# TUM-AVS/Frenetix-Motion-Planner

Measured on AMD Instinct MI355X. Metric: candidate trajectories/sec (30-step horizon), higher is better.
Workload: dtype f64; 1 GPU; BASELINE config3: single agent, 50388 candidates/GPU x 31 samples (19x51x52 grid per GPU), 20 predicted obstacles (prediction cost + OBB collision), SoA TrajectoryBundle materialised (Mode B); candidates_global=50388, candidates_per_gpu=50388, samples=31, reference_knots=400, obstacles=20, parallelism=single GPU, exchange=none (one rank)

## Files before the change

frenetix-motion-planner_amd/csrc/fx_api.hip:

```cpp
#include "fx_context.h"

thread_local char g_err[512] = "";

extern "C" int32_t fx_wait_word(const volatile unsigned long long *word, unsigned long long expected, int32_t timeout_ms) {
    if (!word) return set_err(FX_ERR_INVALID_ARGUMENT, "fx_wait_word: NULL argument");
    for (int spin = 0; spin < 4096; spin++)
        if (__atomic_load_n(word, __ATOMIC_ACQUIRE) == expected) return FX_OK;
    const auto t0 = std::chrono::steady_clock::now();
    const auto limit = std::chrono::milliseconds(timeout_ms < 0 ? 0 : timeout_ms);
    for (;;) {
        for (int spin = 0; spin < 1024; spin++)
            if (__atomic_load_n(word, __ATOMIC_ACQUIRE) == expected) return FX_OK;
        if (std::chrono::steady_clock::now() - t0 >= limit)
            return set_err(FX_ERR_TIMEOUT, "no answer from the device within %d ms (a peer that never joined the collective, or a "
                           "faulted kernel)", timeout_ms);
    }
}

extern "C" {


int32_t fx_abi_version(void) { return FX_ABI_VERSION; }
const char *fx_last_error(void) { return g_err; }

// ... 285 lines not shown
    const int n = (int)std::min<long long>(have, max_n);
    for (int k = 0; k < n; k++) {
        FxContext::TimeSlot &t = c->ring[(c->n_timed - n + k) % FxContext::kTimeRing];
        int rc = fetch_slot(c, t);
        if (rc) return rc;
        if (obst_ms) obst_ms[k] = t.obst_ms;
    }
    *n_out = n;
    return FX_OK;
}
int32_t fx_step_info_ex(const FxContext *c, int64_t *out16) {
    if (!c || !out16) return set_err(FX_ERR_INVALID_ARGUMENT, "fx_step_info_ex: NULL argument");
    int rc = fx_step_info(c, out16);
    if (rc) return rc;
    out16[10] = c->split_step; out16[11] = c->split_CH; out16[12] = c->obs_blocks_step; out16[13] = (int64_t)c->obs_lds_step;
    out16[14] = c->obs_wg_step; out16[15] = c->tail_step | ((int64_t)c->stage_path << 8);
    if (c->step_kernel_step) {
        out16[11] = c->step_CH; out16[12] = (int64_t)c->step_blocks * (FX_BLOCK / 64); out16[13] = (int64_t)c->step_lds; out16[14] = 0;
        out16[15] |= 1 << 16;
    }
    return FX_OK;
}

int32_t fx_set_step_kernel(FxContext *c, int32_t mode, int32_t steps_per_item) {
    if (!c) return set_err(FX_ERR_INVALID_ARGUMENT, "context is NULL");
    if (mode < 0 || mode > 2) return set_err(FX_ERR_INVALID_ARGUMENT, "mode must be 0 (auto), 1 (off: three launches) or 2 (on where applicable)");
    if (steps_per_item != 0 && steps_per_item != 3 && steps_per_item != 5 && steps_per_item != 8)
        return set_err(FX_ERR_INVALID_ARGUMENT, "steps_per_item must be 0 (auto), 3, 5 or 8");
    c->step_kernel_force = mode; c->step_kernel_CH = steps_per_item;
    return FX_OK;
}
// ... 25 lines not shown
```

frenetix-motion-planner_amd/csrc/fx_api_exchange.hip:

```cpp
#include "fx_context.h"

extern "C" {

namespace {
struct Rccl {
    typedef struct { char internal[128]; } UniqueId;
    int (*GetUniqueId)(UniqueId *) = nullptr;
    int (*CommInitRank)(void **, int, UniqueId, int) = nullptr;
    int (*CommDestroy)(void *) = nullptr;
    int (*AllGather)(const void *, void *, size_t, int, void *, hipStream_t) = nullptr;
    int (*CommCount)(void *, int *) = nullptr;
    const char *(*GetErrorString)(int) = nullptr;
    bool ok = false;
};
Rccl *rccl() {
    static Rccl r;
    static std::once_flag once;
    std::call_once(once, [] {
        void *h = dlopen("librccl.so.1", RTLD_NOW | RTLD_LOCAL);
        if (!h) h = dlopen("librccl.so", RTLD_NOW | RTLD_LOCAL);
        if (h) {
            r.GetUniqueId = reinterpret_cast<decltype(r.GetUniqueId)>(dlsym(h, "ncclGetUniqueId"));
            r.CommInitRank = reinterpret_cast<decltype(r.CommInitRank)>(dlsym(h, "ncclCommInitRank"));
            r.CommDestroy = reinterpret_cast<decltype(r.CommDestroy)>(dlsym(h, "ncclCommDestroy"));
// ... 204 lines not shown
    keep_hip(hipSetDevice(c->device), "hipSetDevice");
    if (total > c->gather_cap) {
        double *bigger = nullptr;
        if (hipStreamSynchronize(c->stream) == hipSuccess && hipMalloc(reinterpret_cast<void **>(&bigger), sizeof(double) * (size_t)FX_PUB_MAX) == hipSuccess) {
            if (c->d_gather) { (void)hipFree(c->d_gather); c->dev_bytes -= (int64_t)(sizeof(double) * c->gather_cap); }
            c->d_gather = bigger; c->gather_cap = FX_PUB_MAX; c->dev_bytes += (int64_t)(sizeof(double) * (size_t)FX_PUB_MAX);
        } else {
            (void)hipGetLastError();
            return set_err(FX_ERR_HIP, "fx_step_exchange_topk: no memory for the %zu-element receive buffer", (size_t)FX_PUB_MAX);
        }
    }
    if (c->n_agents > A) keep(set_err(FX_ERR_CAPACITY, "%d uploaded agents but the communicator exchanges %d rows per rank (fx_comm_set_agents)", c->n_agents, A));
    long long *send_idx = reinterpret_cast<long long *>(c->d_xsend + (size_t)A * k);
    bool evaluated = false;
    if (!rc_local) {
        const int rc = fx_evaluate(c);
        keep(rc);
        if (rc == FX_OK) {
            const hipError_t e = fx_launch_topk(c->d_probs, c->n_agents, max_candidates_of(c), k, c->d_topk_scr_cost, c->d_topk_scr_idx, c->d_xsend, send_idx, c->stream);
            keep_hip(e, "fx_launch_topk");
            evaluated = e == hipSuccess;
        }
    }
    const int n_mine = evaluated ? c->n_agents : 0;
    if (c->comm_k_clean != k || c->comm_rows_clean > n_mine) {
        keep_hip(fill_no_survivor(c, n_mine, k), "hipMemcpyAsync");
        c->comm_k_clean = k;
    }
    c->comm_rows_clean = n_mine;
    RCCL_TRY(rccl()->AllGather(c->d_xsend, exchange_recv(c), n,  8, c->comm, c->stream));
    int rc;
// ... 15 lines not shown
```

frenetix-motion-planner_amd/csrc/fx_api_step.hip:

```cpp
#include "fx_context.h"

extern "C" {

int32_t fx_upload_batch(FxContext *c, int32_t n_agents, const FxProblem *probs) {
    if (!c || !probs) return set_err(FX_ERR_INVALID_ARGUMENT, "fx_upload: NULL argument");
    if (n_agents < 1 || n_agents > c->max_agents) return set_err(FX_ERR_CAPACITY, "n_agents=%d exceeds capacity %d", n_agents, c->max_agents);
    if (c->timed_out) return set_err(FX_ERR_TIMEOUT, "an earlier wait on this context timed out (its stream may never drain): destroy it");
    HIP_TRY(hipSetDevice(c->device));
    if (c->in_flight) {
        { HIP_TRY(hipStreamSynchronize(c->stream)); c->tail_work = c->user_stream; }
        c->in_flight = false;
    }
    c->uploaded = c->evaluated = false;
    Arena ar{c->h_in, c->d_in, c->probs_bytes, c->in_bytes};
    size_t bound_need = 0;
    for (int a = 0; a < n_agents; a++) {
        const FxProblem *p = &probs[a];
        if ((p->mode & FX_MODE_ROAD_BOUNDARY) && p->n_bound > 0 && p->bound_bin && p->M > 0)
            bound_need += align_up(sizeof(double) * 4 * (size_t)p->n_bound, 256) + align_up(sizeof(int32_t) * ((size_t)p->M + 1), 256) +
                          align_up(sizeof(int32_t) * (size_t)std::max(p->bound_bin[p->M], 0), 256);
        if (p->n_lane > 0 && p->lane_poly_off && p->lane_ctr_off)
            bound_need += align_up(sizeof(double) * 4 * (size_t)p->n_lane, 256) + 2 * align_up(sizeof(int32_t) * ((size_t)p->n_lane + 1), 256) +
                          align_up(sizeof(double) * 2 * (size_t)std::max(p->lane_poly_off[p->n_lane], 0), 256) +
                          align_up(sizeof(double) * 2 * (size_t)std::max(p->lane_ctr_off[p->n_lane], 0), 256);
// ... 268 lines not shown
            const size_t rb = sizeof(double) * (size_t)S_rec_doubles(S, std::max(p->K, 0));
            if (!deferred && p->K > 0 && p->K <= 64 && rb <= FX_REC_LDS_MAX && (rec_rule_grid || rec_rule_gen)) d.mode |= FX_MODE_INT_REC_LDS;
        }
        all_deferred = all_deferred && deferred;
        if (deferred) {
            d.mode |= FX_MODE_INT_DEFER_OBST;
            const int n_tiles = (int)((C + 63) / 64), NC = (S - 1 + c->split_CH - 1) / c->split_CH;
            const int NC_alloc = std::max(NC, (S - 1 + 2) / 3);
            d.n_blocks = n_tiles;
            c->obs_blocks_step = std::max(c->obs_blocks_step, n_tiles * NC);
            c->obs_tiles_step = std::max(c->obs_tiles_step, n_tiles);
            c->obs_wg_waves = std::max(c->obs_wg_waves, NC);
            d.obs_part = reinterpret_cast<double *>(obs_part_need);
            d.obs_colm = reinterpret_cast<unsigned long long *>(obs_colm_need);
            d.obs_ticket = reinterpret_cast<unsigned int *>(obs_tick_need);
            obs_part_need += (size_t)NC_alloc * (size_t)ld;
            obs_colm_need += (size_t)NC_alloc * (size_t)n_tiles;
            obs_tick_need += (size_t)n_tiles;
        }
        if (block_off + d.n_blocks > c->max_blocks_total)
            return set_err(FX_ERR_CAPACITY, "agent %d: %lld workgroups exceed the partial-result capacity %lld", a,
                           (long long)(block_off + d.n_blocks), (long long)c->max_blocks_total);
        d.part_cost = c->d_part_cost + block_off;
        d.part_idx = c->d_part_idx + block_off;
        d.counters = c->d_counters + (size_t)a * FX_CNT_COUNT;
        d.pkg_out = c->h_pkg_dev + (size_t)a * c->pkg_stride;
        d.pkg_seq = reinterpret_cast<unsigned long long *>(d.pkg_out + c->pkg_stride - 1);
        d.pkg_plane_rows = c->pkg_plane_rows;
        if (d.mode & FX_MODE_WRITE_BUNDLE) {
            if ((uint64_t)ld * 8u >= (1ull << 32))
                return set_err(FX_ERR_CAPACITY, "agent %d: %lld candidates with a materialised bundle (rows are limited to 4 GiB)", a, (long long)C);
// ... 49 lines not shown
            HIP_TRY(hipMemsetAsync(c->d_obs_ticket, 0, sizeof(unsigned int) * n_tick, c->stream));
        }
        if (!c->d_obs_list) {
            int rc;
            if ((rc = dev_alloc(c, &c->d_obs_list, (size_t)c->total_ld))) return rc;
        }
        for (int a = 0; a < n_agents; a++) {
            DevProblem &d = c->h_probs[a];
            if (!(d.mode & FX_MODE_INT_DEFER_OBST)) continue;
            d.obs_part = c->d_obs_part + reinterpret_cast<size_t>(d.obs_part);
            d.obs_colm = c->d_obs_colm + reinterpret_cast<size_t>(d.obs_colm);
            d.obs_ticket = c->d_obs_ticket + reinterpret_cast<size_t>(d.obs_ticket);
            d.obs_list = c->d_obs_list + (d.cost - c->d_cost);
        }
    }
    c->step_kernel_ok = c->step_kernel_force == 2 && c->split_step && all_deferred && c->use_grid && c->G_step == 2 && c->wsplit_step &&
                        c->block_step == FX_BLOCK && c->wpe_step == 2 && c->any_bundle && !c->any_obst && !c->any_extra && c->wt_step &&
                        c->obs_blocks_step > 0 && c->K_max_step <= 64;
    c->last_live = -1;
    c->n_agents = n_agents;
    c->in_used = ar.off;
    c->dirty_lo = (size_t)-1; c->dirty_hi = 0; c->probs_dirty = false;
    {
        const size_t up = (ar.off + 15) & ~(size_t)15;
        if (up <= c->in_bytes && host_stage_allowed(c, up))
            host_stage(c, 0, up);
        else if (c->stage_mode == 2 || (c->stage_mode != 1 && up <= FX_STAGE_KERNEL_MAX && up <= c->in_bytes)) {
            HIP_TRY(fx_launch_stage(c->h_in_dev, c->d_in, up, c->stream));
            c->stage_path = 2;
        } else {
// ... 44 lines not shown
    if (timed && !attached) HIP_TRY(hipEventRecord(ts->e0, c->stream));
    c->seq++;
    c->fused_step = c->fuse_enabled && c->fusable_step && c->eval_launched;
    c->pkg_step = c->package_enabled && c->any_bundle;
    double *winner = c->dev_winner ? c->dev_winner : (c->pkg_step ? c->d_winner_own : nullptr);
    const bool tail_kernel = FX_TAIL_IN_KERNEL(c->G_step, c->any_extra);
    if (c->fused_step && c->count_step && !tail_kernel) c->fused_step = false;
    c->tail_step = 0;
    if (c->fused_step && tail_kernel) {
        if (c->count_step) c->tail_step |= FX_TAIL_COUNT;
        if (c->pkg_step && c->wt_step) c->tail_step |= FX_TAIL_PACKAGE;
    }
    const bool pkg_in_tail = (c->tail_step & FX_TAIL_PACKAGE) != 0;
    FuseArgs fuse{c->fused_step ? c->h_counters_dev : nullptr, c->seq, winner, (int32_t)((uint32_t)c->K_max_step | (c->tail_step << 16))};
    c->step_kernel_step = false;
    if (c->step_kernel_ok && !c->fused_step && c->eval_launched) {
        int64_t c_max = 0;
        for (int a = 0; a < c->n_agents; a++) c_max = std::max(c_max, c->slots[a].C);
        const int64_t live_est = c->last_live >= 0 ? std::min(c->last_live, c_max) : (2 * c_max + 2) / 3;
        const int tiles_est = (int)std::max<int64_t>(1, (live_est + 63) / 64);
        int best_CH = 0, best_blocks = 0, best_score = 1 << 30;
        size_t best_lds = 0;
        static const int chs[3] = {3, 5, 8};
        for (int q = 0; q < 3; q++) {
            const int CH = chs[q];
            if (c->step_kernel_CH && c->step_kernel_CH != CH) continue;
            const size_t lds = std::max(c->lds_step, (size_t)(FX_BLOCK / 64) * sizeof(double) * 6 * (size_t)CH * (size_t)c->K_max_step);
            int cap = 0;
            {
                static std::mutex mu;
// ... 43 lines not shown
        else
            HIP_TRY(fx_launch_eval(c->d_probs, c->n_agents, c->max_blocks_step,
                                   sizeof(double) * ((size_t)c->M_max_step * FX_REF_FIELDS + FX_TP * (size_t)c->S_max_step +
                                                     (((size_t)c->M_max_step + 1) & ~(size_t)1)) + c->gen_rec_lds,
                                   c->G_step, c->any_bundle, c->any_obst, c->any_extra, c->wpe_step, k0, k1, fuse, c->stream));
    }
    if (timed && !attached) HIP_TRY(hipEventRecord(ts->e_eval, c->stream));
    if (timed) ts->obst_timed = false;
    if (c->split_step && c->obs_blocks_step > 0) {
        const bool t_obs = timed && c->timing == FX_TIMING_KERNEL;
        const char *wg_env = getenv("FX_OBST_WG");
        const int wg_mode = wg_env ? (atoi(wg_env) ? 2 : 1) : ((int64_t)c->obs_tiles_step * c->n_agents <= 1024 ? 2 : 1);
        const size_t lds_wg = align_up((size_t)c->obs_wg_waves * (c->obs_lds_step + 64 * sizeof(double) + sizeof(unsigned long long)), 16);
        const bool wg = wg_mode == 2 && c->obs_wg_waves >= 1 && c->obs_wg_waves <= 16 && lds_wg <= (size_t)160 * 1024 - 1024;
        c->obs_wg_step = wg ? c->obs_wg_waves : 0;
        HIP_TRY(fx_launch_obstacle(c->d_probs, c->n_agents, c->obs_blocks_step, wg ? lds_wg : c->obs_lds_step, c->split_CH,
                                   t_obs ? ts->e_obs0 : nullptr, t_obs ? ts->e_obs1 : nullptr, c->stream, wg ? c->obs_wg_waves : 0,
                                   c->obs_tiles_step));
        if (timed) ts->obst_timed = t_obs;
    }
    if (!c->fused_step) {
        int64_t c_max = 0;
        for (int a = 0; a < c->n_agents; a++) c_max = std::max(c_max, c->slots[a].C);
        HIP_TRY(fx_launch_select(c->d_probs, c->n_agents, c_max, c->h_counters_dev, c->seq, winner, c->pkg_step ? c->h_pkg_dev : nullptr,
                                 c->pkg_stride, c->pkg_plane_rows, c->stream));
    } else if (c->pkg_step && !pkg_in_tail) {
        HIP_TRY(fx_launch_package(c->d_probs, c->n_agents, winner, c->h_pkg_dev, c->pkg_stride, c->pkg_plane_rows, c->seq, c->stream));
    }
    const bool one_launch = c->fused_step && (!c->pkg_step || pkg_in_tail);
    if (timed && !one_launch) HIP_TRY(hipEventRecord(ts->e_end, c->stream));
    if (timed) { ts->fused = one_launch; c->n_timed++; }
    c->timed_step = timed;
    c->evaluated = true;
    c->in_flight = true;
    return FX_OK;
}
// ... 274 lines not shown
```

frenetix-motion-planner_amd/csrc/fx_context.h:

```cpp
#pragma once

#include <hip/hip_runtime.h>

#include <algorithm>
#include <chrono>
#include <cmath>
#include <cstdarg>
#include <cstdio>
#include <cstdlib>
#include <cstring>
#include <atomic>

#include <map>
#include <memory>
#include <mutex>
#include <new>
#include <thread>
#include <tuple>
#include <vector>
#include <dlfcn.h>
#include <fcntl.h>
#include <unistd.h>

#include "fx_device.h"

extern "C" hipError_t fx_launch_eval(const DevProblem *d_probs, int n_agents, int max_blocks, size_t lds_bytes, int G,
                                     bool bundle, bool obst, bool extra, int wpe, hipEvent_t ev_start, hipEvent_t ev_stop,
                                     FuseArgs fuse, hipStream_t stream);
extern "C" hipError_t fx_launch_eval_grid(const DevProblem *d_probs, int n_agents, int max_blocks, int block_size,
                                          size_t lds_bytes, int G, bool bundle, bool obst, int wpe, bool wsplit,
                                          hipEvent_t ev_start, hipEvent_t ev_stop, FuseArgs fuse, hipStream_t stream);
extern "C" hipError_t fx_launch_obstacle(const DevProblem *d_probs, int n_agents, int max_items, size_t lds_bytes, int CH,
                                         hipEvent_t ev_start, hipEvent_t ev_stop, hipStream_t stream, int wg_waves, int max_tiles);
extern "C" hipError_t fx_step_kernel_capacity(int CH, size_t lds_bytes, int *blocks_out);
extern "C" hipError_t fx_launch_step(const DevProblem *d_probs, int n_agents, int blocks, size_t lds_bytes, int CH, hipEvent_t ev_start,
                                     hipEvent_t ev_stop, FuseArgs fuse, StepArgs sa, hipStream_t stream);
extern "C" hipError_t fx_launch_select(const DevProblem *d_probs, int n_agents, int64_t max_candidates, unsigned long long *host_result,
                                       unsigned long long seq, double *dev_winner, double *host_pkg, int pkg_stride, int pkg_plane_rows,
                                       hipStream_t stream);
extern "C" hipError_t fx_launch_math_test(int n, const double *x, double *at, double *sn, double *cs, hipStream_t stream);
extern "C" hipError_t fx_launch_publish(const double *src, int n, double *host_dst, unsigned long long *host_seq,
                                        unsigned long long seq, hipStream_t stream);
extern "C" hipError_t fx_launch_stage(const void *src_mapped, void *dst, size_t bytes, hipStream_t stream);
extern "C" hipError_t fx_launch_package(const DevProblem *d_probs, int n_agents, const double *winner, double *host_pkg, int stride,
                                        int plane_rows, unsigned long long seq, hipStream_t stream);
extern "C" hipError_t fx_launch_topk(const DevProblem *d_probs, int n_agents, int64_t max_candidates, int k, double *scr_cost, long long *scr_idx,
                                     double *out_cost, long long *out_idx, hipStream_t stream);

// ... 124 lines not shown
    size_t in_used = 0;
    size_t dirty_lo = (size_t)-1, dirty_hi = 0;
    bool probs_dirty = false;
    int max_blocks_step = 0, M_max_step = 0, S_max_step = 0, K_max_step = 0;
    int G_step = 1, wpe_step = 2;
    int G_force = 0, wpe_force = 0;
    int variant_force = 0;
    int block_force = 0;
    int wsplit_force = 0;
    int obst_force = 0;
    int obst_CH = 0;
    bool split_step = false;
    int split_CH = 3, obs_blocks_step = 0;
    int obs_wg_waves = 0, obs_tiles_step = 0;
    int obs_wg_step = 0;
    size_t obs_lds_step = 0;
    int step_kernel_force = 0;
    int step_kernel_CH = 0;
    bool step_kernel_ok = false;
    bool step_kernel_step = false;
    int step_blocks = 0, step_CH = 0;
    size_t step_lds = 0;
    int64_t last_live = -1;
    unsigned long long *d_bar = nullptr;
    unsigned long long bar_base = 0;
    int store_force = 0;
    bool wsplit_step = false;
    int block_step = FX_BLOCK;
    bool use_grid = false;
    size_t lds_step = 0;
// ... 262 lines not shown
```

frenetix-motion-planner_amd/csrc/fx_device.h:

```cpp
#pragma once
#include <hip/hip_runtime.h>
#include <stdint.h>

#include "../../include/fxplan.h"

#define FX_BLOCK 256
#define FX_MODE_INT_STORE_WT (1u << 30)
#define FX_MODE_INT_DEFER_OBST (1u << 29)
#define FX_MODE_INT_REC_LDS (1u << 28)
#define FX_HOT_STRIDE 10
#define FX_HOT_PRE 4
#define FX_TP 14
#define FX_REF_FIELDS 8
#define FX_MAX_SAMPLES 128
#define FX_REC_LDS_MAX (48 * 1024)
__host__ __device__ inline int S_rec_doubles(int S, int K) { return S * K * 12; }

struct DevProblem {
    int32_t N, S;
    uint32_t mode;
    int32_t low_vel_mode;
    double dt;
    double x0_lon[3], x0_lat[3];
    double x0_orientation, v_des;
// ... 165 lines not shown
#define FX_MSTAMP(k) do { } while (0)
#endif

#define FX_COEFF_ROWS 13
#define FX_PKG_TAIL (12 + FX_NUM_COSTS + 6)

enum {
    FX_CNT_RETURNED = 0, FX_CNT_FEASIBLE, FX_CNT_HIST0,
    FX_CNT_BEST_IDX = FX_CNT_HIST0 + FX_NUM_REASONS, FX_CNT_BEST_COST, FX_CNT_COLLISIONS, FX_CNT_COUNT
};

#define FX_DCNT_TICKET FX_CNT_BEST_IDX
#define FX_DCNT_LIVE FX_CNT_BEST_COST
#define FX_TAIL_COUNT 1u
#define FX_TAIL_PACKAGE 2u
#define FX_TAIL_IN_KERNEL(G, EXTRA) ((G) >= 4 || (EXTRA))
struct FuseArgs {
    unsigned long long *host_result;
    unsigned long long seq;
    double *dev_winner;
    int32_t k_max;
    __host__ __device__ uint32_t tail() const { return (uint32_t)k_max >> 16; }
    __host__ __device__ int32_t kmax() const { return k_max & 0xffff; }
};

struct StepArgs {
    unsigned long long *bar;
    unsigned long long bar_base;
    unsigned long long *host_result;
    unsigned long long seq;
// ... 22 lines not shown
```

frenetix-motion-planner_amd/csrc/fx_kernels.hip:

```cpp
#include <hip/hip_ext.h>

#include <atomic>

#include "fx_eval_kernel.h"
#include "fx_eval_grid_kernel.h"
#include "fx_obstacle_kernel.h"
#include "fx_step_kernel.h"
#include "fx_risk_kernel.h"

using fxk::wave_count;

#if defined(__HIP_DEVICE_COMPILE__) && !defined(__gfx950__) && !defined(__gfx942__) && !defined(__gfx90a__)
#error "libfxplan's kernels are written for gfx950 (row_bcast DPP controls, wave64): build with --offload-arch=gfx950"
#endif

#define FX_MAX_DEVICES 64
static inline int fx_device_slot() {
    int d = 0;
    if (hipGetDevice(&d) != hipSuccess || d < 0) d = 0;
    return d % FX_MAX_DEVICES;
}

#ifdef FX_CULL_STATS
__device__ unsigned long long fx_cull_stats[16];
// ... 395 lines not shown
    }
    switch (G) {
    case 32: FX_BO(32, 2, false);
    case 16: FX_BO(16, 2, false);
    case 8: FX_W(8, false);
    case 4: FX_W(4, false);
    case 2: FX_W(2, false);
    default: FX_W(1, false);
    }
#undef FX_W
#undef FX_BO
#undef FX_LAUNCH
}

extern "C" hipError_t fx_launch_obstacle(const DevProblem *d_probs, int n_agents, int max_items, size_t lds_bytes, int CH,
                                         hipEvent_t ev_start, hipEvent_t ev_stop, hipStream_t stream, int wg_waves, int max_tiles) {
#define FX_LAUNCH(CHv)                                                                                                                \
    do {                                                                                                                            \
        if (wg_waves > 0) {                                                                                                         \
            static std::atomic<size_t> lds_set_[FX_MAX_DEVICES];                                                                    \
            std::atomic<size_t> &hw_ = lds_set_[fx_device_slot()];                                                                  \
            if (lds_bytes > 48 * 1024 && lds_bytes > hw_.load(std::memory_order_relaxed)) {                                         \
                hipError_t e_ = hipFuncSetAttribute(reinterpret_cast<const void *>(&fxk::fx_obstacle_kernel<CHv, 4, true>),          \
                                                    hipFuncAttributeMaxDynamicSharedMemorySize, (int)lds_bytes);                    \
                if (e_ != hipSuccess) return e_;                                                                                    \
                hw_.store(lds_bytes, std::memory_order_relaxed);                                                                    \
            }                                                                                                                       \
            hipExtLaunchKernelGGL((fxk::fx_obstacle_kernel<CHv, 4, true>), dim3(max_tiles, n_agents), dim3(64 * wg_waves), lds_bytes, stream, \
                                  ev_start, ev_stop, 0, d_probs);                                                                   \
        } else {                                                                                                                    \
            hipExtLaunchKernelGGL((fxk::fx_obstacle_kernel<CHv, 4, false>), dim3(max_items, n_agents), dim3(64), lds_bytes, stream, ev_start, \
                                  ev_stop, 0, d_probs);                                                                             \
        }                                                                                                                           \
        return hipGetLastError();                                                                                                   \
    } while (0)
    if (CH == 2) FX_LAUNCH(2);
    if (CH == 3) FX_LAUNCH(3);
    if (CH == 5) FX_LAUNCH(5);
#undef FX_LAUNCH
    return hipErrorInvalidValue;
}

#define FX_STEP_CASES(X) X(3) X(5) X(8)
extern "C" hipError_t fx_step_kernel_capacity(int CH, size_t lds_bytes, int *blocks_out) {
    int dev = 0, cus = 0, per_cu = 0;
    hipError_t e = hipGetDevice(&dev);
    if (e != hipSuccess) return e;
// ... 69 lines not shown
```

frenetix-motion-planner_amd/csrc/fx_obstacle_kernel.h:

```cpp
#pragma once

#include "fx_eval_kernel.h"

namespace fxk {

struct ObsEntry {
    double l11, l12, l22;
    fx_d2 cc;
};
template <class HotPtr>
__device__ __forceinline__ ObsEntry obs_load(HotPtr hot_i, const fx_d2 *cc_i, int k) {
    const auto q = hot_i + (size_t)k * FX_HOT_STRIDE;
    ObsEntry e;
    e.l11 = q[FX_HOT_L11]; e.l12 = q[FX_HOT_L12]; e.l22 = q[FX_HOT_L22];
    e.cc = cc_i[k];
    return e;
}
__device__ __forceinline__ double obs_msq(const ObsEntry &e, double xr, double yr) {
    const double u = fma(e.l11, xr, fma(e.l12, yr, -e.cc.x));
    const double w = fma(e.l22, yr, -e.cc.y);
    const double m = fma(u, u, w * w);
    return m * m;
}
__device__ __forceinline__ double obs_four(double a, double b, double c, double d) {
    const double ab = a * b, cd = c * d;
    const double num = fma(a + b, cd, (c + d) * ab);
    return num * rcp_pred(ab * cd);
}

#ifndef FX_OBST_WG_WPE
#define FX_OBST_WG_WPE 1
#endif
template <int CH, bool WG, bool COH>
__device__ __forceinline__ void fx_obstacle_body(const DevProblem &P, double *__restrict__ lds_all, const int tile, const int chunk,
                                                 const long long n_live_known = -1) {
    static_assert(!COH || !WG, "the one-launch step runs single-wave items");
    auto LD = [](auto p) { return *p; };
    auto ST = [](auto p, auto v) { if (COH) st_agent(p, v); else *p = v; };
    const uint32_t mode = P.mode;
    if (!(mode & FX_MODE_INT_DEFER_OBST)) return;
    const int S = P.S, K = P.K;
    const int NC = (S - 1 + CH - 1) / CH;
    const int64_t C = P.C, ld = P.ld;
    const int n_wave = WG ? (int)(blockDim.x >> 6) : 1;
    const int64_t c0 = (int64_t)tile * 64;
    if (c0 >= C) return;
    const int lane = threadIdx.x & 63;
    double *__restrict__ lds_dyn = lds_all + (WG ? (size_t)chunk * 6 * CH * (size_t)K : 0);
    double *__restrict__ sh_part = lds_all + (size_t)n_wave * 6 * CH * (size_t)K;
    unsigned long long *__restrict__ sh_colm = reinterpret_cast<unsigned long long *>(sh_part + (size_t)n_wave * 64);
    FX_OSTAMP(0);
    const FX_GLOBAL unsigned long long *cnt_live = as_global(P.counters) + FX_DCNT_LIVE;
    unsigned long long n_live_raw = 0ULL;
    int32_t g_listed = 0;
    if (!COH) {
        n_live_raw = *cnt_live;
        g_listed = as_global(P.obs_list)[c0 + lane];
    } else {
        n_live_raw = (unsigned long long)n_live_known;
        g_listed = ld_agent(as_global(P.obs_list) + (c0 + lane));
    }

    const int i_a = 1 + chunk * CH, i_b = min(S, i_a + CH);
    const int64_t ps = (int64_t)S * ld;
    const FX_GLOBAL double *__restrict__ pl = as_global(P.planes);
    const bool col_mode = (mode & FX_MODE_COLLISION) != 0 && K > 0;
    const auto hot_a = as_table<COH>(P.obs_hot) + (size_t)i_a * K * FX_HOT_STRIDE;
    fx_d2 *__restrict__ cc_tab = reinterpret_cast<fx_d2 *>(lds_dyn);
    double *__restrict__ circ_tab = lds_dyn + 2 * (size_t)CH * K;
    const int n_e = max((i_b - i_a) * K, 0);
    double hv[2][6];
#pragma unroll
    for (int u = 0; u < 2; u++) {
        const int e = max(min(lane + 64 * u, n_e - 1), 0);
        const auto q = hot_a + (size_t)e * FX_HOT_STRIDE;
        const bool on = n_e > 0 && K > 0;
        hv[u][0] = on ? q[FX_HOT_CU] : 0.0; hv[u][1] = on ? q[FX_HOT_CW] : 0.0;
        hv[u][2] = on ? q[FX_HOT_HX2] : 0.0; hv[u][3] = on ? q[FX_HOT_HY2] : 0.0; hv[u][4] = on ? q[FX_HOT_HR2] : 0.0; hv[u][5] = on ? q[FX_HOT_CK] : 0.0;
    }
    auto park_tables = [&]() {
#pragma unroll
        for (int u = 0; u < 2; u++) {
// ... 27 lines not shown
    const uint32_t f = LD(as_global(P.flags) + g);
    double xs[CH + 1], ys[CH + 1], ts[CH + 1];
#pragma unroll
    for (int j = 0; j <= CH; j++) {
        const int i = min(i_a - 1 + j, S - 1);
        xs[j] = LD(pl + ((int64_t)FX_PL_X * ps + (int64_t)i * ld + g));
        ys[j] = LD(pl + ((int64_t)FX_PL_Y * ps + (int64_t)i * ld + g));
        ts[j] = col_mode ? LD(pl + ((int64_t)FX_PL_THETA * ps + (int64_t)i * ld + g)) : 0.0;
    }
    double pre_cost = 0.0, pre_tail = 0.0;
    if (WG && chunk == 0) {
        pre_cost = LD(as_global(P.cost) + g);
        pre_tail = LD(as_global(P.cost_tail) + g);
    }
    const int64_t n_live = (int64_t)n_live_raw;
    if (c0 >= n_live) {
        if (chunk == 0 && lane == 0) {
            ST(as_global(P.part_cost) + tile, (double)INFINITY);
            ST(as_global(P.part_idx) + tile, (int64_t)0x7fffffffffffffffLL);
        }
        return;
    }
    const bool act = c0 + lane < n_live;
    park_tables();

    int n_pred = -1;
    double w_pred = 0.0;
    bool has_tail = false;
    for (int n = 0; n < P.n_cost; n++)
        if (P.cost_id[n] == FX_COST_PREDICTION) { n_pred = n; w_pred = P.cost_w[n]; has_tail = n + 1 < P.n_cost; }
    const bool do_pred = n_pred >= 0 && K > 0 && wave_any_bit(act && (f & FX_FLAG_COSTED));
    const bool do_col = col_mode && wave_any_bit(act && (f & FX_FLAG_SELECTABLE));
    FX_OSTAMP(1);

    double acc = 0.0;
    bool collided = false;
    const bool work = do_pred || do_col;
    if (!work && chunk != 0) return;
    if (work && chunk < NC) {
        const auto rec = as_table<COH>(P.obs_rec);
        const auto pmask = as_table<COH>(P.obs_pmask);
        const auto hmask = as_table<COH>(P.obs_hmask);
        const double ox = P.hot_origin[0], oy = P.hot_origin[1];
        const double wb = P.veh.wb_rear_axle, half_len = P.veh.length / 2, half_wid = P.veh.width / 2;
        const double gap_margin = P.hot_gap_margin;
        const float cull_r0 = (float)((fabs(wb) * 2.41422 + 1.41423 * sqrt(half_len * half_len + half_wid * half_wid)) * 1.00001);
        const unsigned long long full = K >= 64 ? ~0ULL : ((1ULL << K) - 1ULL);
        const int kl = min(lane, K - 1);
        __builtin_amdgcn_fence(__ATOMIC_RELEASE, "wavefront");
        __builtin_amdgcn_wave_barrier();
        __builtin_amdgcn_fence(__ATOMIC_ACQUIRE, "wavefront");
        double sn_prev = 0.0, cs_prev = 1.0;
        bool have_prev = false;
        FX_OSTAMP(2);
#pragma unroll
        for (int j = 1; j <= CH; j++) {
            const int i = i_a + j - 1;
// ... 94 lines not shown
                }
            }
        }
    }
    FX_OSTAMP(4);
    FX_GLOBAL double *__restrict__ part = as_global(P.obs_part);
    FX_GLOBAL unsigned long long *__restrict__ colm = as_global(P.obs_colm);
    FX_GLOBAL unsigned int *__restrict__ ticket = as_global(P.obs_ticket);
    const int64_t n_tiles = (C + 63) / 64;
    if (WG) {
        if (work) {
            sh_part[chunk * 64 + lane] = acc;
            const unsigned long long cm = __builtin_amdgcn_ballot_w64(collided);
            if (lane == 0) sh_colm[chunk] = cm;
            __syncthreads();
            if (chunk != 0) return;
        }
    } else if (work) {
        if (act) __hip_atomic_store(part + (int64_t)chunk * ld + g_raw, acc, __ATOMIC_RELAXED, __HIP_MEMORY_SCOPE_AGENT);
        const unsigned long long cm = __builtin_amdgcn_ballot_w64(collided);
        if (lane == 0) __hip_atomic_store(colm + (int64_t)chunk * n_tiles + tile, cm, __ATOMIC_RELAXED, __HIP_MEMORY_SCOPE_AGENT);
        asm volatile("s_waitcnt vmcnt(0)" ::: "memory");
        unsigned int t = 0;
        if (lane == 0) t = __hip_atomic_fetch_add(ticket + tile, 1u, __ATOMIC_RELAXED, __HIP_MEMORY_SCOPE_AGENT);
        t = __builtin_amdgcn_readfirstlane(t);
        FX_OSTAMP(5);
        if (t != (unsigned)(NC - 1)) return;
        if (lane == 0) __hip_atomic_store(ticket + tile, 0u, __ATOMIC_RELAXED, __HIP_MEMORY_SCOPE_AGENT);
    }
    double pred = 0.0;
    unsigned long long cmask = 0ULL;
    if (work && WG) {
        for (int q = 0; q < NC; q++) {
            pred += sh_part[q * 64 + lane];
            cmask |= sh_colm[q];
        }
    } else if (work) {
        for (int q = 0; q < NC; q++) {
            pred += __hip_atomic_load(part + (int64_t)q * ld + g_raw, __ATOMIC_RELAXED, __HIP_MEMORY_SCOPE_AGENT);
            cmask |= __hip_atomic_load(colm + (int64_t)q * n_tiles + tile, __ATOMIC_RELAXED, __HIP_MEMORY_SCOPE_AGENT);
        }
    }
// ... 14 lines not shown
        fl |= FX_FLAG_COLLISION;
        if (act) ST(as_global(P.flags) + g, fl);
    }
    const bool eligible = act && selectable && !(fl & (FX_FLAG_COLLISION | FX_FLAG_BOUNDARY)) && total == total;
    const double bc = eligible ? total : INFINITY;
    double m = bc;
#pragma unroll
    for (int off = 32; off >= 1; off >>= 1) m = fmin(m, __shfl_xor(m, off));
    long long bi = (eligible && bc == m) ? (long long)(g_raw + P.g_base) : 0x7fffffffffffffffLL;
#pragma unroll
    for (int off = 32; off >= 1; off >>= 1) { const long long o = __shfl_xor(bi, off); bi = o < bi ? o : bi; }
    if (lane == 0) {
        ST(as_global(P.part_cost) + tile, m);
        ST(as_global(P.part_idx) + tile, (int64_t)bi);
    }
    FX_OSTAMP(15);
}

template <int CH, int WPS, bool WG = false>
__global__ __launch_bounds__(WG ? 1024 : 64, WG ? FX_OBST_WG_WPE : WPS) void fx_obstacle_kernel(const DevProblem *__restrict__ probs) {
    extern __shared__ __attribute__((aligned(16))) double lds_all[];
    const DevProblem &P = probs[blockIdx.y];
    const int NC = (P.S - 1 + CH - 1) / CH;
    const int tile = WG ? (int)blockIdx.x : (int)(blockIdx.x / NC);
    const int chunk = WG ? (int)__builtin_amdgcn_readfirstlane(threadIdx.x >> 6) : (int)(blockIdx.x - tile * NC);
    fx_obstacle_body<CH, WG, false>(P, lds_all, tile, chunk);
}

}
```

frenetix-motion-planner_amd/engine.py:

```python
import ctypes as C
from typing import List, Optional, Sequence

import numpy as np

from . import _abi
from ._lib import check, lib
from .problem import PlanInputs


def build_obstacle_hulls(n_pred, pos, yaw, length, width) -> np.ndarray:
    pos = np.ascontiguousarray(pos, dtype=np.float64)
    yaw = np.ascontiguousarray(yaw, dtype=np.float64)
    out = np.zeros((max(int(n_pred) - 1, 1), 6))
    n = C.c_int32(0)
    check(lib().fx_build_obstacle_hulls(int(n_pred), pos.ctypes.data_as(C.POINTER(C.c_double)),
                                        yaw.ctypes.data_as(C.POINTER(C.c_double)), float(length), float(width),
                                        out.ctypes.data_as(C.POINTER(C.c_double)), C.byref(n)))
    return out[:n.value]


def _build_obstacle_hulls_batch(n_use, pos, yaw, length, width, hull, nhull):
    K, P = pos.shape[0], pos.shape[1]
    length, width = np.ascontiguousarray(length, dtype=np.float64), np.ascontiguousarray(width, dtype=np.float64)
    check(lib().fx_build_obstacle_hulls_batch(K, P, n_use.ctypes.data, pos.ctypes.data, yaw.ctypes.data, length.ctypes.data,
# ... 216 lines not shown

    def set_step_kernel(self, mode: int = 0, steps_per_item: int = 0):
        check(lib().fx_set_step_kernel(self._ctx, int(mode), int(steps_per_item)))
        self._resident_key = None
        self._resident_keys = None

    def step_info(self) -> dict:
        v = np.zeros(16, np.int64)
        check(lib().fx_step_info_ex(self._ctx, v.ctypes.data))
        keys = ("grid_kernel", "lanes_per_candidate", "waves_per_simd", "block", "wave_split", "fused_selection", "blocks", "agents",
                "package", "lds_bytes", "obstacle_kernel", "obstacle_steps_per_item", "obstacle_items", "obstacle_lds_bytes",
                "obstacle_workgroup_waves", "tail")
        info = dict(zip(keys, (int(x) for x in v)))
        info["staging"] = ("none", "dma", "kernel", "host_writes")[(info["tail"] >> 8) & 3]
        info["step_kernel"] = (info["tail"] >> 16) & 1
        info["tail"] &= 0xff
        return info

    def obstacle_kernel_times(self, max_n: int = 256):
        ob = np.zeros(max_n, dtype=np.float64)
        n = C.c_int32(0)
        check(lib().fx_read_obstacle_kernel_times(self._ctx, max_n, ob.ctypes.data_as(C.POINTER(C.c_double)), C.byref(n)))
        return ob[:n.value]

    @property
    def last_obstacle_kernel_ms(self) -> float:
        return float(lib().fx_last_obstacle_kernel_ms(self._ctx))

    TIMING = {"off": 0, "stream": 1, "kernel": 2}

# ... 393 lines not shown
```

Before: 592.2 million trajectories/s.

## Fold final selection into obstacle kernel via last-block ticket tail

When the obstacle stage runs in workgroup mode with deferred obstacles and no fused selection, each tile now writes a compact per-tile record: best cost and index, low and high bounds, and counts of collided candidates below its tile minimum. The last workgroup to finish, found through an atomic ticket, reduces these records to the winner and collision count, writes the host result and package, and resets the counters. This removes the separate selection kernel launch. In exchange it adds per-tile stores, a ticket atomic, coherent loads, and a serial single-wave tail. It is disabled during exchange and can be turned off with the FX_OBST_FOLD environment variable.

```diff
diff --git a/frenetix-motion-planner_amd/csrc/fx_api.hip b/frenetix-motion-planner_amd/csrc/fx_api.hip
--- a/frenetix-motion-planner_amd/csrc/fx_api.hip
+++ b/frenetix-motion-planner_amd/csrc/fx_api.hip
@@ -323,7 +323,7 @@
     int rc = fx_step_info(c, out16);
     if (rc) return rc;
     out16[10] = c->split_step; out16[11] = c->split_CH; out16[12] = c->obs_blocks_step; out16[13] = (int64_t)c->obs_lds_step;
-    out16[14] = c->obs_wg_step; out16[15] = c->tail_step | ((int64_t)c->stage_path << 8);
+    out16[14] = c->obs_wg_step; out16[15] = c->tail_step | ((int64_t)c->stage_path << 8) | ((int64_t)c->obs_fold_step << 17);
     if (c->step_kernel_step) {
         out16[11] = c->step_CH; out16[12] = (int64_t)c->step_blocks * (FX_BLOCK / 64); out16[13] = (int64_t)c->step_lds; out16[14] = 0;
         out16[15] |= 1 << 16;
diff --git a/frenetix-motion-planner_amd/csrc/fx_api_exchange.hip b/frenetix-motion-planner_amd/csrc/fx_api_exchange.hip
--- a/frenetix-motion-planner_amd/csrc/fx_api_exchange.hip
+++ b/frenetix-motion-planner_amd/csrc/fx_api_exchange.hip
@@ -242,7 +242,9 @@
     long long *send_idx = reinterpret_cast<long long *>(c->d_xsend + (size_t)A * k);
     bool evaluated = false;
     if (!rc_local) {
+        c->fold_block = true;
         const int rc = fx_evaluate(c);
+        c->fold_block = false;
         keep(rc);
         if (rc == FX_OK) {
             const hipError_t e = fx_launch_topk(c->d_probs, c->n_agents, max_candidates_of(c), k, c->d_topk_scr_cost, c->d_topk_scr_idx, c->d_xsend, send_idx, c->stream);
diff --git a/frenetix-motion-planner_amd/csrc/fx_api_step.hip b/frenetix-motion-planner_amd/csrc/fx_api_step.hip
--- a/frenetix-motion-planner_amd/csrc/fx_api_step.hip
+++ b/frenetix-motion-planner_amd/csrc/fx_api_step.hip
@@ -306,7 +306,7 @@
             d.obs_part = reinterpret_cast<double *>(obs_part_need);
             d.obs_colm = reinterpret_cast<unsigned long long *>(obs_colm_need);
             d.obs_ticket = reinterpret_cast<unsigned int *>(obs_tick_need);
-            obs_part_need += (size_t)NC_alloc * (size_t)ld;
+            obs_part_need += std::max((size_t)NC_alloc * (size_t)ld, (size_t)n_tiles * FX_FOLD_TILE_WORDS);
             obs_colm_need += (size_t)NC_alloc * (size_t)n_tiles;
             obs_tick_need += (size_t)n_tiles;
         }
@@ -386,6 +386,7 @@
             d.obs_list = c->d_obs_list + (d.cost - c->d_cost);
         }
     }
+    c->all_deferred_step = all_deferred;
     c->step_kernel_ok = c->step_kernel_force == 2 && c->split_step && all_deferred && c->use_grid && c->G_step == 2 && c->wsplit_step &&
                         c->block_step == FX_BLOCK && c->wpe_step == 2 && c->any_bundle && !c->any_obst && !c->any_extra && c->wt_step &&
                         c->obs_blocks_step > 0 && c->K_max_step <= 64;
@@ -460,6 +461,7 @@
     const bool pkg_in_tail = (c->tail_step & FX_TAIL_PACKAGE) != 0;
     FuseArgs fuse{c->fused_step ? c->h_counters_dev : nullptr, c->seq, winner, (int32_t)((uint32_t)c->K_max_step | (c->tail_step << 16))};
     c->step_kernel_step = false;
+    c->obs_fold_step = false;
     if (c->step_kernel_ok && !c->fused_step && c->eval_launched) {
         int64_t c_max = 0;
         for (int a = 0; a < c->n_agents; a++) c_max = std::max(c_max, c->slots[a].C);
@@ -533,12 +535,17 @@
         const size_t lds_wg = align_up((size_t)c->obs_wg_waves * (c->obs_lds_step + 64 * sizeof(double) + sizeof(unsigned long long)), 16);
         const bool wg = wg_mode == 2 && c->obs_wg_waves >= 1 && c->obs_wg_waves <= 16 && lds_wg <= (size_t)160 * 1024 - 1024;
         c->obs_wg_step = wg ? c->obs_wg_waves : 0;
+        const char *fold_env = getenv("FX_OBST_FOLD");
+        c->obs_fold_step = wg && c->all_deferred_step && !c->fused_step && !c->fold_block && (!fold_env || atoi(fold_env) != 0);
+        const FuseArgs fold{c->obs_fold_step ? c->h_counters_dev : nullptr, c->seq, winner,
+                            (int32_t)((uint32_t)c->K_max_step | ((c->pkg_step ? FX_TAIL_PACKAGE : 0u) << 16))};
         HIP_TRY(fx_launch_obstacle(c->d_probs, c->n_agents, c->obs_blocks_step, wg ? lds_wg : c->obs_lds_step, c->split_CH,
                                    t_obs ? ts->e_obs0 : nullptr, t_obs ? ts->e_obs1 : nullptr, c->stream, wg ? c->obs_wg_waves : 0,
-                                   c->obs_tiles_step));
+                                   c->obs_tiles_step, fold));
         if (timed) ts->obst_timed = t_obs;
     }
-    if (!c->fused_step) {
+    if (c->obs_fold_step) {
+    } else if (!c->fused_step) {
         int64_t c_max = 0;
         for (int a = 0; a < c->n_agents; a++) c_max = std::max(c_max, c->slots[a].C);
         HIP_TRY(fx_launch_select(c->d_probs, c->n_agents, c_max, c->h_counters_dev, c->seq, winner, c->pkg_step ? c->h_pkg_dev : nullptr,
diff --git a/frenetix-motion-planner_amd/csrc/fx_context.h b/frenetix-motion-planner_amd/csrc/fx_context.h
--- a/frenetix-motion-planner_amd/csrc/fx_context.h
+++ b/frenetix-motion-planner_amd/csrc/fx_context.h
@@ -31,7 +31,8 @@
                                           size_t lds_bytes, int G, bool bundle, bool obst, int wpe, bool wsplit,
                                           hipEvent_t ev_start, hipEvent_t ev_stop, FuseArgs fuse, hipStream_t stream);
 extern "C" hipError_t fx_launch_obstacle(const DevProblem *d_probs, int n_agents, int max_items, size_t lds_bytes, int CH,
-                                         hipEvent_t ev_start, hipEvent_t ev_stop, hipStream_t stream, int wg_waves, int max_tiles);
+                                         hipEvent_t ev_start, hipEvent_t ev_stop, hipStream_t stream, int wg_waves, int max_tiles,
+                                         FuseArgs fold);
 extern "C" hipError_t fx_step_kernel_capacity(int CH, size_t lds_bytes, int *blocks_out);
 extern "C" hipError_t fx_launch_step(const DevProblem *d_probs, int n_agents, int blocks, size_t lds_bytes, int CH, hipEvent_t ev_start,
                                      hipEvent_t ev_stop, FuseArgs fuse, StepArgs sa, hipStream_t stream);
@@ -186,6 +187,9 @@
     int split_CH = 3, obs_blocks_step = 0;
     int obs_wg_waves = 0, obs_tiles_step = 0;
     int obs_wg_step = 0;
+    bool all_deferred_step = false;
+    bool fold_block = false;
+    bool obs_fold_step = false;
     size_t obs_lds_step = 0;
     int step_kernel_force = 0;
     int step_kernel_CH = 0;
diff --git a/frenetix-motion-planner_amd/csrc/fx_device.h b/frenetix-motion-planner_amd/csrc/fx_device.h
--- a/frenetix-motion-planner_amd/csrc/fx_device.h
+++ b/frenetix-motion-planner_amd/csrc/fx_device.h
@@ -203,6 +203,8 @@
 #define FX_DCNT_LIVE FX_CNT_BEST_COST
 #define FX_TAIL_COUNT 1u
 #define FX_TAIL_PACKAGE 2u
+#define FX_FOLD_REC 8
+#define FX_FOLD_TILE_WORDS (FX_FOLD_REC + 2 * 64)
 #define FX_TAIL_IN_KERNEL(G, EXTRA) ((G) >= 4 || (EXTRA))
 struct FuseArgs {
     unsigned long long *host_result;
diff --git a/frenetix-motion-planner_amd/csrc/fx_kernels.hip b/frenetix-motion-planner_amd/csrc/fx_kernels.hip
--- a/frenetix-motion-planner_amd/csrc/fx_kernels.hip
+++ b/frenetix-motion-planner_amd/csrc/fx_kernels.hip
@@ -433,7 +433,9 @@
 }
 
 extern "C" hipError_t fx_launch_obstacle(const DevProblem *d_probs, int n_agents, int max_items, size_t lds_bytes, int CH,
-                                         hipEvent_t ev_start, hipEvent_t ev_stop, hipStream_t stream, int wg_waves, int max_tiles) {
+                                         hipEvent_t ev_start, hipEvent_t ev_stop, hipStream_t stream, int wg_waves, int max_tiles,
+                                         FuseArgs fold) {
+    if (wg_waves <= 0) fold = FuseArgs{nullptr, 0ULL, nullptr, 0};
 #define FX_LAUNCH(CHv)                                                                                                                \
     do {                                                                                                                            \
         if (wg_waves > 0) {                                                                                                         \
@@ -446,10 +448,10 @@
                 hw_.store(lds_bytes, std::memory_order_relaxed);                                                                    \
             }                                                                                                                       \
             hipExtLaunchKernelGGL((fxk::fx_obstacle_kernel<CHv, 4, true>), dim3(max_tiles, n_agents), dim3(64 * wg_waves), lds_bytes, stream, \
-                                  ev_start, ev_stop, 0, d_probs);                                                                   \
+                                  ev_start, ev_stop, 0, d_probs, fold);                                                                   \
         } else {                                                                                                                    \
             hipExtLaunchKernelGGL((fxk::fx_obstacle_kernel<CHv, 4, false>), dim3(max_items, n_agents), dim3(64), lds_bytes, stream, ev_start, \
-                                  ev_stop, 0, d_probs);                                                                             \
+                                  ev_stop, 0, d_probs, fold);                                                                             \
         }                                                                                                                           \
         return hipGetLastError();                                                                                                   \
     } while (0)
diff --git a/frenetix-motion-planner_amd/csrc/fx_obstacle_kernel.h b/frenetix-motion-planner_amd/csrc/fx_obstacle_kernel.h
--- a/frenetix-motion-planner_amd/csrc/fx_obstacle_kernel.h
+++ b/frenetix-motion-planner_amd/csrc/fx_obstacle_kernel.h
@@ -1,6 +1,7 @@
 #pragma once
 
 #include "fx_eval_kernel.h"
+#include "fx_select.h"
 
 namespace fxk {
 
@@ -32,19 +33,33 @@
 #define FX_OBST_WG_WPE 1
 #endif
 template <int CH, bool WG, bool COH>
-__device__ __forceinline__ void fx_obstacle_body(const DevProblem &P, double *__restrict__ lds_all, const int tile, const int chunk,
-                                                 const long long n_live_known = -1) {
+__device__ __forceinline__ bool fx_obstacle_body(const DevProblem &P, double *__restrict__ lds_all, const int tile, const int chunk,
+                                                 const long long n_live_known = -1, const bool fold_req = false,
+                                                 int64_t *n_live_out = nullptr) {
     static_assert(!COH || !WG, "the one-launch step runs single-wave items");
+    const bool fold = WG && fold_req;
     auto LD = [](auto p) { return *p; };
-    auto ST = [](auto p, auto v) { if (COH) st_agent(p, v); else *p = v; };
+    auto ST = [&](auto p, auto v) { if (COH || fold) st_agent(p, v); else *p = v; };
+    auto last_ticket = [&]() -> bool {
+        if (!fold || chunk != 0) return false;
+        drain_stores();
+        unsigned long long t = 0ULL;
+        if ((threadIdx.x & 63) == 0)
+            t = __hip_atomic_fetch_add(as_global(P.counters) + FX_DCNT_TICKET, 1ULL, __ATOMIC_RELAXED, __HIP_MEMORY_SCOPE_AGENT);
+        t = __shfl(t, 0);
+        return t == (unsigned long long)(gridDim.x - 1);
+    };
     const uint32_t mode = P.mode;
-    if (!(mode & FX_MODE_INT_DEFER_OBST)) return;
+    if (!(mode & FX_MODE_INT_DEFER_OBST)) return false;
     const int S = P.S, K = P.K;
     const int NC = (S - 1 + CH - 1) / CH;
     const int64_t C = P.C, ld = P.ld;
     const int n_wave = WG ? (int)(blockDim.x >> 6) : 1;
     const int64_t c0 = (int64_t)tile * 64;
-    if (c0 >= C) return;
+    if (c0 >= C) {
+        if (n_live_out) *n_live_out = (int64_t)*(as_global(P.counters) + FX_DCNT_LIVE);
+        return last_ticket();
+    }
     const int lane = threadIdx.x & 63;
     double *__restrict__ lds_dyn = lds_all + (WG ? (size_t)chunk * 6 * CH * (size_t)K : 0);
     double *__restrict__ sh_part = lds_all + (size_t)n_wave * 6 * CH * (size_t)K;
@@ -65,7 +80,7 @@
     const int64_t ps = (int64_t)S * ld;
     const FX_GLOBAL double *__restrict__ pl = as_global(P.planes);
     const bool col_mode = (mode & FX_MODE_COLLISION) != 0 && K > 0;
-    const auto hot_a = as_table<COH>(P.obs_hot) + (size_t)i_a * K * FX_HOT_STRIDE;
+    const auto hot_a = as_table<COH || WG>(P.obs_hot) + (size_t)i_a * K * FX_HOT_STRIDE;
     fx_d2 *__restrict__ cc_tab = reinterpret_cast<fx_d2 *>(lds_dyn);
     double *__restrict__ circ_tab = lds_dyn + 2 * (size_t)CH * K;
     const int n_e = max((i_b - i_a) * K, 0);
@@ -123,12 +138,13 @@
         pre_tail = LD(as_global(P.cost_tail) + g);
     }
     const int64_t n_live = (int64_t)n_live_raw;
+    if (n_live_out) *n_live_out = n_live;
     if (c0 >= n_live) {
         if (chunk == 0 && lane == 0) {
             ST(as_global(P.part_cost) + tile, (double)INFINITY);
             ST(as_global(P.part_idx) + tile, (int64_t)0x7fffffffffffffffLL);
         }
-        return;
+        return last_ticket();
     }
     const bool act = c0 + lane < n_live;
     park_tables();
@@ -145,11 +161,11 @@
     double acc = 0.0;
     bool collided = false;
     const bool work = do_pred || do_col;
-    if (!work && chunk != 0) return;
+    if (!work && chunk != 0) return false;
     if (work && chunk < NC) {
-        const auto rec = as_table<COH>(P.obs_rec);
-        const auto pmask = as_table<COH>(P.obs_pmask);
-        const auto hmask = as_table<COH>(P.obs_hmask);
+        const auto rec = as_table<COH || WG>(P.obs_rec);
+        const auto pmask = as_table<COH || WG>(P.obs_pmask);
+        const auto hmask = as_table<COH || WG>(P.obs_hmask);
         const double ox = P.hot_origin[0], oy = P.hot_origin[1];
         const double wb = P.veh.wb_rear_axle, half_len = P.veh.length / 2, half_wid = P.veh.width / 2;
         const double gap_margin = P.hot_gap_margin;
@@ -274,7 +290,7 @@
             const unsigned long long cm = __builtin_amdgcn_ballot_w64(collided);
             if (lane == 0) sh_colm[chunk] = cm;
             __syncthreads();
-            if (chunk != 0) return;
+            if (chunk != 0) return false;
         }
     } else if (work) {
         if (act) __hip_atomic_store(part + (int64_t)chunk * ld + g_raw, acc, __ATOMIC_RELAXED, __HIP_MEMORY_SCOPE_AGENT);
@@ -285,7 +301,7 @@
         if (lane == 0) t = __hip_atomic_fetch_add(ticket + tile, 1u, __ATOMIC_RELAXED, __HIP_MEMORY_SCOPE_AGENT);
         t = __builtin_amdgcn_readfirstlane(t);
         FX_OSTAMP(5);
-        if (t != (unsigned)(NC - 1)) return;
+        if (t != (unsigned)(NC - 1)) return false;
         if (lane == 0) __hip_atomic_store(ticket + tile, 0u, __ATOMIC_RELAXED, __HIP_MEMORY_SCOPE_AGENT);
     }
     double pred = 0.0;
@@ -330,17 +346,148 @@
         ST(as_global(P.part_cost) + tile, m);
         ST(as_global(P.part_idx) + tile, (int64_t)bi);
     }
+    if (fold) {
+        const bool hit = act && selectable && (fl & FX_FLAG_COLLISION);
+        const long long key_i = g_raw + P.g_base;
+        const bool below = hit && fx_lex_less(total, key_i, m, bi);
+        const unsigned long long b_all = __builtin_amdgcn_ballot_w64(hit), b_low = __builtin_amdgcn_ballot_w64(below);
+        const int n_tiles_a = (int)((C + 63) / 64);
+        FX_GLOBAL unsigned long long *recw = reinterpret_cast<FX_GLOBAL unsigned long long *>(as_global(P.obs_part));
+        FX_GLOBAL double *slot_c = reinterpret_cast<FX_GLOBAL double *>(recw + (size_t)n_tiles_a * FX_FOLD_REC + (size_t)tile * 128);
+        FX_GLOBAL long long *slot_i = reinterpret_cast<FX_GLOBAL long long *>(slot_c + 64);
+        double lo = INFINITY, hi = -INFINITY;
+        if (b_low) {
+            const int pos = (int)__builtin_amdgcn_mbcnt_hi((uint32_t)(b_low >> 32), __builtin_amdgcn_mbcnt_lo((uint32_t)b_low, 0u));
+            if (below) { st_agent(slot_c + pos, total); st_agent(slot_i + pos, key_i); }
+            lo = below ? total : INFINITY;
+            hi = below ? total : -INFINITY;
+#pragma unroll
+            for (int off = 32; off >= 1; off >>= 1) { lo = fmin(lo, __shfl_xor(lo, off)); hi = fmax(hi, __shfl_xor(hi, off)); }
+        }
+        unsigned long long w = (unsigned long long)__popcll(b_low) | ((unsigned long long)__popcll(b_all) << 32);
+        if (lane == 0) w = (unsigned long long)__double_as_longlong(m);
+        if (lane == 1) w = (unsigned long long)bi;
+        if (lane == 2) w = (unsigned long long)__double_as_longlong(lo);
+        if (lane == 3) w = (unsigned long long)__double_as_longlong(hi);
+        if (lane < 5) st_agent(recw + (size_t)tile * FX_FOLD_REC + lane, w);
+    }
     FX_OSTAMP(15);
+    return last_ticket();
+}
+
+__device__ __forceinline__ void fx_fold_tail(const DevProblem &P, const FuseArgs fold, const int64_t n_live) {
+    const int lane = threadIdx.x & 63, agent = (int)blockIdx.y;
+    const int64_t C = P.C;
+    const int nt = (int)((min(n_live, C) + 63) / 64);
+    const int n_tiles_a = (int)((C + 63) / 64);
+    const FX_GLOBAL unsigned long long *recw = reinterpret_cast<const FX_GLOBAL unsigned long long *>(as_global(P.obs_part));
+    const FX_GLOBAL unsigned long long *slots = recw + (size_t)n_tiles_a * FX_FOLD_REC;
+    unsigned long long cnt = 0ULL;
+    if (lane < FX_CNT_BEST_IDX) cnt = as_global(P.counters)[lane];
+    constexpr int UA = 8, UB = 4;
+    double bc = INFINITY;
+    long long bi = 0x7fffffffffffffffLL;
+    for (int t0 = lane; t0 < nt; t0 += 64 * UA) {
+        unsigned long long c[UA];
+        long long ix[UA];
+#pragma unroll
+        for (int u = 0; u < UA; u++) {
+            const int t = min(t0 + 64 * u, nt - 1);
+            c[u] = ld_agent(recw + (size_t)t * FX_FOLD_REC);
+            ix[u] = (long long)ld_agent(recw + (size_t)t * FX_FOLD_REC + 1);
+        }
+#pragma unroll
+        for (int u = 0; u < UA; u++)
+            if (fx_lex_less(__longlong_as_double((long long)c[u]), ix[u], bc, bi)) { bc = __longlong_as_double((long long)c[u]); bi = ix[u]; }
+    }
+    fx_lex_wave_min(bc, bi);
+    const bool none = bi == 0x7fffffffffffffffLL;
+    unsigned int mine = 0;
+    if (P.mode & FX_MODE_COLLISION) {
+        for (int b0 = 0; b0 < nt; b0 += 64 * UB) {
+            const int t0 = b0 + lane;
+            unsigned long long cw[UB];
+            double lo[UB], hi[UB];
+#pragma unroll
+            for (int u = 0; u < UB; u++) {
+                const int t = t0 + 64 * u;
+                const size_t r = (size_t)min(t, nt - 1) * FX_FOLD_REC;
+                cw[u] = t < nt ? ld_agent(recw + r + 4) : 0ULL;
+                lo[u] = none ? 0.0 : __longlong_as_double((long long)ld_agent(recw + r + 2));
+                hi[u] = none ? 0.0 : __longlong_as_double((long long)ld_agent(recw + r + 3));
+            }
+            bool straddle[UB];
+#pragma unroll
+            for (int u = 0; u < UB; u++) {
+                const unsigned n_low = (unsigned)(cw[u] & 0xffffffffULL);
+                if (none) mine += (unsigned)(cw[u] >> 32);
+                else if (n_low != 0 && hi[u] < bc) mine += n_low;
+                straddle[u] = !none && n_low != 0 && !(hi[u] < bc) && !(lo[u] > bc);
+            }
+#pragma unroll
+            for (int u = 0; u < UB; u++) {
+                const unsigned n_low = (unsigned)(cw[u] & 0xffffffffULL);
+                unsigned long long sm = __builtin_amdgcn_ballot_w64(straddle[u]);
+                while (sm) {
+                    int tk[4], nk[4];
+#pragma unroll
+                    for (int q = 0; q < 4; q++) {
+                        const int src = sm ? __builtin_ctzll(sm) : -1;
+                        if (sm) sm &= sm - 1;
+                        tk[q] = src >= 0 ? __builtin_amdgcn_readlane(t0 + 64 * u, src) : -1;
+                        nk[q] = src >= 0 ? __builtin_amdgcn_readlane((int)n_low, src) : 0;
+                    }
+                    double kc[4];
+                    long long ki[4];
+#pragma unroll
+                    for (int q = 0; q < 4; q++) {
+                        const bool on = lane < nk[q];
+                        const FX_GLOBAL unsigned long long *sl = slots + (size_t)max(tk[q], 0) * 128 + (on ? lane : 0);
+                        kc[q] = on ? __longlong_as_double((long long)ld_agent(sl)) : 0.0;
+                        ki[q] = on ? (long long)ld_agent(sl + 64) : 0LL;
+                    }
+#pragma unroll
+                    for (int q = 0; q < 4; q++)
+                        if (lane < nk[q] && fx_lex_less(kc[q], ki[q], bc, bi)) mine++;
+                }
+            }
+        }
+#pragma unroll
+        for (int off = 32; off >= 1; off >>= 1) mine += __shfl_xor(mine, off);
+    }
+    unsigned long long *out = fold.host_result + (size_t)agent * (FX_CNT_COUNT + 1);
+    {
+        unsigned long long w = cnt;
+        if (lane == FX_CNT_BEST_IDX) w = none ? ~0ULL : (unsigned long long)bi;
+        if (lane == FX_CNT_BEST_COST) w = none ? 0ULL : (unsigned long long)__double_as_longlong(bc);
+        if (lane == FX_CNT_COLLISIONS) w = mine;
+        if (lane < FX_CNT_COUNT) put_host(out + lane, w);
+    }
+    if (lane < FX_CNT_BEST_IDX) as_global(P.counters)[lane] = 0ULL;
+    if (lane == 0) {
+        if (fold.dev_winner) {
+            fold.dev_winner[2 * agent] = none ? INFINITY : bc;
+            reinterpret_cast<long long *>(fold.dev_winner)[2 * agent + 1] = none ? -1 : bi;
+        }
+        __hip_atomic_store(&P.counters[FX_DCNT_TICKET], 0ULL, __ATOMIC_RELAXED, __HIP_MEMORY_SCOPE_AGENT);
+        as_global(P.counters)[FX_DCNT_LIVE] = 0ULL;
+    }
+    double *pkg = (fold.tail() & FX_TAIL_PACKAGE) ? P.pkg_out : nullptr;
+    if (pkg) fx_package_gather<true>(P, none ? -1LL : bi, pkg, P.pkg_plane_rows, lane, 64);
+    else drain_stores();
+    if (lane == 0 || (lane == 1 && pkg)) st_host(lane == 0 ? out + FX_CNT_COUNT : P.pkg_seq, fold.seq);
 }
 
 template <int CH, int WPS, bool WG = false>
-__global__ __launch_bounds__(WG ? 1024 : 64, WG ? FX_OBST_WG_WPE : WPS) void fx_obstacle_kernel(const DevProblem *__restrict__ probs) {
+__global__ __launch_bounds__(WG ? 1024 : 64, WG ? FX_OBST_WG_WPE : WPS) void fx_obstacle_kernel(const DevProblem *__restrict__ probs,
+                                                                                                const FuseArgs fold) {
     extern __shared__ __attribute__((aligned(16))) double lds_all[];
     const DevProblem &P = probs[blockIdx.y];
     const int NC = (P.S - 1 + CH - 1) / CH;
     const int tile = WG ? (int)blockIdx.x : (int)(blockIdx.x / NC);
     const int chunk = WG ? (int)__builtin_amdgcn_readfirstlane(threadIdx.x >> 6) : (int)(blockIdx.x - tile * NC);
-    fx_obstacle_body<CH, WG, false>(P, lds_all, tile, chunk);
-}
-
-}
+    int64_t n_live = 0;
+    if (fx_obstacle_body<CH, WG, false>(P, lds_all, tile, chunk, -1, WG && fold.host_result != nullptr, &n_live)) fx_fold_tail(P, fold, n_live);
+}
+
+}
diff --git a/frenetix-motion-planner_amd/engine.py b/frenetix-motion-planner_amd/engine.py
--- a/frenetix-motion-planner_amd/engine.py
+++ b/frenetix-motion-planner_amd/engine.py
@@ -254,6 +254,7 @@
         info = dict(zip(keys, (int(x) for x in v)))
         info["staging"] = ("none", "dma", "kernel", "host_writes")[(info["tail"] >> 8) & 3]
         info["step_kernel"] = (info["tail"] >> 16) & 1
+        info["obstacle_fold"] = (info["tail"] >> 17) & 1
         info["tail"] &= 0xff
         return info
 
```

Result: slower. 468.4 million trajectories/s (median of 2 runs) (-20.9%).
